# MetaHG/mitsuba2

Hardware: AMD Instinct MI355X
Metric: Msample/s, cbox 1024x1024@256spp per GPU, path integrator (max_depth=-1, rr_depth=5) (higher is better)
Workload: dtype f32

## Files before the change

### mitsuba2_amd/csrc/device_scene.h

```cpp
#pragma once
#include "device_math.h"
#include "device_bsdf.h"
#include "device_envmap.h"
#include "flat_worklist.h"

namespace mtsamd {

constexpr uint32_t kLeafFlag = 0x80000000u;
constexpr uint32_t kLeafCountShift = 27;
constexpr uint32_t kLeafStartMask = (1u << kLeafCountShift) - 1u;
constexpr uint32_t kNoPrim = 0xffffffffu;

#ifndef MTS_BVH4
#define MTS_BVH4 1
#endif
#if MTS_BVH4
typedef uint2 StackEntry;
typedef uint64_t StackRaw;
#else
typedef uint32_t StackEntry;
typedef uint32_t StackRaw;
#endif


struct DevShape { int32_t bsdf; int32_t emitter; uint32_t flags; uint32_t first_prim; };
constexpr uint32_t kShapeHasNormals = 1u, kShapeHasUV = 2u;
struct DevTexture {
    const float *data; int32_t w, h; uint32_t grad_offset, kind;
    float uvm[6];
    float c0[3], c1[3];
    float mean;
};
struct DevEmitter {
    float r, g, b; uint32_t shape;
    uint32_t first_prim, n_prims; float area_sum, area_norm;
    uint32_t valid_lo, valid_hi; uint32_t pad0, pad1;
    float c0, c1, c2, d65_scale;
// ... 22 lines not shown
    const float *tri_uv;
    const uint32_t *prim_shape;
    const DevShape *shapes;
    const DevBsdf *bsdfs;
    const DevEmitter *emitters; uint32_t n_emitters;
    uint32_t n_shapes, n_bsdfs;
    const DevTexture *textures; uint32_t n_textures;
    const float *area_pmf, *area_cdf;
    const float4 *flat_recs;
    const float4 *flat_pairs;
    uint32_t flat, n_pairs, n_clusters;
    int32_t env_emitter;
    const DevEnvmap *envmap;
    uint32_t general;
};
constexpr uint32_t kFlatMaxPrims = 64;

struct LdsView {
    const float4 *nodes;
    const float4 *tris;
    uint32_t *stack;
    uint32_t stride;
    StackEntry *spill;
    uint32_t spill_stride, stack_lds_depth;
    const float4 *flat;
    const float4 *pairs;
    const float4 *clusters;
    const DevShape *shapes;
    const DevBsdf *bsdfs;
    const DevEmitter *emitters;
    const float *pmf, *cdf;
    uint32_t *wl;
};

#ifndef MTS_FLAT_WORKLIST
#define MTS_FLAT_WORKLIST 1
#endif
#ifndef MTS_FLAT_WL_ROUNDS
#define MTS_FLAT_WL_ROUNDS 5
#endif
constexpr uint32_t kWlItems = 64u * MTS_FLAT_WL_ROUNDS;
constexpr uint32_t kWlWords = 128u + kWlItems / 2u;

inline uint32_t flat_shape_count(const SceneView &sv) { return sv.n_shapes; }

template <bool FLAT>
MTS_DEV LdsView lds_stage(const SceneView &sv, float4 *smem) {
    LdsView l = {};
    l.stride = blockDim.x;
    if (FLAT) {
        float4 *f = smem;
        for (uint32_t i = threadIdx.x; i < 4u * sv.n_prims; i += blockDim.x) f[i] = sv.flat_recs[i];
        l.flat = f;
        float4 *pr = f + 4u * sv.n_prims;
        for (uint32_t i = threadIdx.x; i < 5u * sv.n_pairs; i += blockDim.x) pr[i] = sv.flat_pairs[i];
        if (threadIdx.x < 5u) pr[5u * sv.n_pairs + threadIdx.x] = make_float4(0.0f, 0.0f, 0.0f, 0.0f);
        l.pairs = pr;
        float4 *cl = pr + 5u * sv.n_pairs + 5u;
        for (uint32_t i = threadIdx.x; i < 2u * sv.n_clusters; i += blockDim.x) cl[i] = sv.flat_pairs[5u * sv.n_pairs + i];
        l.clusters = cl;
        uint32_t *w = reinterpret_cast<uint32_t *>(cl + 2u * sv.n_clusters);
        const uint32_t n_sh = (sizeof(DevShape) / 4u) * sv.n_shapes, n_bs = (sizeof(DevBsdf) / 4u) * sv.n_bsdfs,
                       n_em = (sizeof(DevEmitter) / 4u) * sv.n_emitters;
        const uint32_t *g_sh = reinterpret_cast<const uint32_t *>(sv.shapes), *g_bs = reinterpret_cast<const uint32_t *>(sv.bsdfs),
                       *g_em = reinterpret_cast<const uint32_t *>(sv.emitters);
        for (uint32_t i = threadIdx.x; i < n_sh; i += blockDim.x) w[i] = g_sh[i];
        l.shapes = reinterpret_cast<const DevShape *>(w); w += n_sh;
        for (uint32_t i = threadIdx.x; i < n_bs; i += blockDim.x) w[i] = g_bs[i];
        l.bsdfs = reinterpret_cast<const DevBsdf *>(w); w += n_bs;
        for (uint32_t i = threadIdx.x; i < n_em; i += blockDim.x) w[i] = g_em[i];
        l.emitters = reinterpret_cast<const DevEmitter *>(w); w += n_em;
        float *fw = reinterpret_cast<float *>(w);
        for (uint32_t i = threadIdx.x; i < sv.n_prims; i += blockDim.x) { fw[i] = sv.area_pmf[i]; fw[sv.n_prims + i] = sv.area_cdf[i]; }
        l.pmf = fw; l.cdf = fw + sv.n_prims;
        const uint32_t wl_off = (uint32_t) (reinterpret_cast<uint32_t *>(fw + 2u * sv.n_prims) - reinterpret_cast<uint32_t *>(smem));
        l.wl = MTS_FLAT_WORKLIST ? reinterpret_cast<uint32_t *>(smem) + ((wl_off + 1u) & ~1u) : nullptr;
    } else {
        float4 *n = smem;
        float4 *t = n + 4u * sv.lds_nodes;
        for (uint32_t i = threadIdx.x; i < 4u * sv.lds_nodes; i += blockDim.x) n[i] = sv.nodes[i];
        for (uint32_t i = threadIdx.x; i < 3u * sv.lds_slots; i += blockDim.x) t[i] = sv.tris[i];
        l.nodes = n; l.tris = t;
        l.stack = reinterpret_cast<uint32_t *>(t + 3u * sv.lds_slots);
    }
    __syncthreads();
    return l;
}
inline size_t lds_bytes(const SceneView &sv, uint32_t block) {
    if (sv.flat)
        return (size_t) 64 * sv.n_prims + (size_t) 80 * (sv.n_pairs + 1) + (size_t) 32 * sv.n_clusters + sizeof(DevShape) * sv.n_shapes + sizeof(DevBsdf) * sv.n_bsdfs +
               sizeof(DevEmitter) * sv.n_emitters + (size_t) 8 * sv.n_prims +
               (MTS_FLAT_WORKLIST ? 4u + (size_t) 4 * kWlWords * (block / 64u) : 0u);
    return (size_t) 64 * sv.lds_nodes + (size_t) 48 * sv.lds_slots + sizeof(StackEntry) * sv.stack_depth * block;
}

#ifndef MTS_FLAT_UNROLL
#define MTS_FLAT_UNROLL 1
#endif
#ifndef MTS_FLAT_PREFETCH
#define MTS_FLAT_PREFETCH 1
#endif

struct Hit { float t; uint32_t prim; float u, v; };

MTS_DEV bool tri_test(f3 p0, f3 e1, f3 e2, f3 o, f3 d, float mint, float maxt, float &u, float &v, float &t) {
    f3 pvec = cross(d, e2);
    float inv_det = rcp(dot(e1, pvec));
    f3 tvec = o - p0;
    u = dot(tvec, pvec) * inv_det;
    bool ok = (u >= 0.0f) && (u <= 1.0f);
    f3 qvec = cross(tvec, e1);
    v = dot(d, qvec) * inv_det;
    ok = ok && (v >= 0.0f) && (u + v <= 1.0f);
    t = dot(e2, qvec) * inv_det;
    return ok && (t >= mint) && (t <= maxt);
}

MTS_DEV float clamp_mag(float r) { return fabsf(r) <= 3.0e38f ? r : copysignf(3.0e38f, r); }
MTS_DEV float clamp_mag33(float r) { return fabsf(r) <= 1.0e33f ? r : copysignf(1.0e33f, r); }
MTS_DEV float clamp_inv(float d) {
    float r = 1.0f / d;
    return fabsf(r) <= 3.0e38f ? r : copysignf(3.0e38f, d);
}

constexpr uint32_t kNoNode = 0x7fffffffu;
// ... 531 lines not shown
    if (MTS_FLAT_LATE_UV && best_prim != kNoPrim) flat_hit_uv(lds, o, d, best_prim, bu, bv);
    hit.t = best; hit.prim = best_prim; hit.u = bu; hit.v = bv;
    return best_prim != kNoPrim;
}

MTS_DEV bool traverse_flat_clustered_any(const SceneView &sv, const LdsView &lds, f3 o, f3 d, float mint, float maxt, uint32_t &tri_tests) {
    bool any = false;
    if (!(MTS_CULL_STATS & 2)) tri_tests += sv.n_prims;
    const v2f ox = splat(o.x), oy = splat(o.y), oz = splat(o.z), dx = splat(d.x), dy = splat(d.y), dz = splat(d.z);
    const f3 inv = mk3(clamp_inv(d.x), clamp_inv(d.y), clamp_inv(d.z));
    const float4 *rec = lds.pairs;
    for (uint32_t c = 0; c < sv.n_clusters; ++c) {
        const float4 lo = lds.clusters[2u * c], hi = lds.clusters[2u * c + 1u];
        const uint32_t n = __float_as_uint(lo.w);
        const float ax = (lo.x - o.x) * inv.x, bx = (hi.x - o.x) * inv.x;
        const float ay = (lo.y - o.y) * inv.y, by = (hi.y - o.y) * inv.y;
        const float az = (lo.z - o.z) * inv.z, bz = (hi.z - o.z) * inv.z;
        const float tn = fmaxf(fmaxf(fminf(ax, bx), fminf(ay, by)), fmaxf(fminf(az, bz), mint));
        const float tf = fminf(fminf(fmaxf(ax, bx), fmaxf(ay, by)), fminf(fmaxf(az, bz), maxt));
        if (__ballot(!any && tn <= tf) == 0ull) { rec += 5u * n; continue; }
        if (MTS_CULL_STATS & 2) tri_tests += 2u * n;
        for (uint32_t i = 0; i < n; ++i) {
            const float4 q0 = rec[0], q1 = rec[1], q2 = rec[2], q3 = rec[3], q4 = rec[4];
            rec += 5;
            const PairUvt r = pair_test(q0, q1, q2, q3, q4, ox, oy, oz, dx, dy, dz);
            const bool ok_a = tri_accept(r.u.x, r.v.x, r.uv.x, r.t.x, mint, maxt);
            const bool ok_b = tri_accept(r.u.y, r.v.y, r.uv.y, r.t.y, mint, maxt);
            any = any || ok_a || ok_b;
        }
    }
    return any;
}

static_assert(kFlatMaxPrims <= 64u, "a pair mask is 32 bits");
template <bool ANY>
MTS_DEV bool traverse_flat_worklist(const SceneView &sv, const LdsView &lds, f3 o, f3 d, float mint, float maxt, Hit &hit, uint32_t &tri_tests) {
    const uint64_t active = __ballot(1);
    const uint32_t n_act = (uint32_t) __popcll(active), lane = lane_id(), rank = mask_rank(active);
    const f3 inv = mk3(clamp_inv(d.x), clamp_inv(d.y), clamp_inv(d.z));
    uint32_t pairs = 0u, first = 0u;
    for (uint32_t c = 0; c < sv.n_clusters; ++c) {
        const float4 lo = lds.clusters[2u * c], hi = lds.clusters[2u * c + 1u];
        const uint32_t n = __float_as_uint(lo.w);
        const float ax = (lo.x - o.x) * inv.x, bx = (hi.x - o.x) * inv.x;
        const float ay = (lo.y - o.y) * inv.y, by = (hi.y - o.y) * inv.y;
        const float az = (lo.z - o.z) * inv.z, bz = (hi.z - o.z) * inv.z;
        const float tn = fmaxf(fmaxf(fminf(ax, bx), fminf(ay, by)), fmaxf(fminf(az, bz), mint));
        const float tf = fminf(fminf(fmaxf(ax, bx), fmaxf(ay, by)), fminf(fmaxf(az, bz), maxt));
        const uint32_t bits = (uint32_t) ((1ull << n) - 1ull) << first;
        pairs |= tn <= tf ? bits : 0u;
        first += n;
    }
    const uint32_t cnt = (uint32_t) __popc(pairs);
    uint32_t pos = 0u, total = 0u;
#pragma unroll
    for (uint32_t b = 0; b < 6u; ++b) {
        const uint64_t m = __ballot((cnt >> b) & 1u);
        pos += mask_rank(m) << b; total += (uint32_t) __popcll(m) << b;
    }
    if (total > kWlItems || total > MTS_FLAT_WL_ROUNDS * n_act) return traverse_flat<ANY>(sv, lds, o, d, mint, maxt, hit, tri_tests);
    constexpr bool kRealCount = (MTS_CULL_STATS & (ANY ? 2 : 1)) != 0;
    if (!kRealCount) tri_tests += sv.n_prims;
    uint32_t *ws = lds.wl + (threadIdx.x >> 6) * kWlWords;
    unsigned long long *key = reinterpret_cast<unsigned long long *>(ws);
    uint16_t *tbl = reinterpret_cast<uint16_t *>(ws + 128u);
    if (ANY) ws[lane] = 0u;
    else key[lane] = kWlNoKey;
    wl_push_items(tbl, pos, pairs, lane);
    __builtin_amdgcn_fence(__ATOMIC_RELEASE, "wavefront");
    __builtin_amdgcn_wave_barrier();
    __builtin_amdgcn_fence(__ATOMIC_ACQUIRE, "wavefront");
    for (uint32_t j0 = 0u; j0 < total; j0 += n_act) {
        const uint32_t j = j0 + rank;
        const uint32_t item = j < total ? (uint32_t) tbl[j] : wl_item(lane, sv.n_pairs);
        const uint32_t owner = wl_item_owner(item), pair = wl_item_pair(item);
        const int addr = (int) (owner << 2);
        const float rox = __int_as_float(__builtin_amdgcn_ds_bpermute(addr, __float_as_int(o.x)));
        const float roy = __int_as_float(__builtin_amdgcn_ds_bpermute(addr, __float_as_int(o.y)));
        const float roz = __int_as_float(__builtin_amdgcn_ds_bpermute(addr, __float_as_int(o.z)));
        const float rdx = __int_as_float(__builtin_amdgcn_ds_bpermute(addr, __float_as_int(d.x)));
        const float rdy = __int_as_float(__builtin_amdgcn_ds_bpermute(addr, __float_as_int(d.y)));
        const float rdz = __int_as_float(__builtin_amdgcn_ds_bpermute(addr, __float_as_int(d.z)));
        const float rmint = __int_as_float(__builtin_amdgcn_ds_bpermute(addr, __float_as_int(mint)));
        const float rmaxt = __int_as_float(__builtin_amdgcn_ds_bpermute(addr, __float_as_int(maxt)));
        const float4 *rec = lds.pairs + 5u * pair;
        const float4 q0 = rec[0], q1 = rec[1], q2 = rec[2], q3 = rec[3], q4 = rec[4];
        const PairUvt r = pair_test(q0, q1, q2, q3, q4, splat(rox), splat(roy), splat(roz), splat(rdx), splat(rdy), splat(rdz));
        const bool ok_a = tri_accept(r.u.x, r.v.x, r.uv.x, r.t.x, rmint, rmaxt);
        const bool ok_b = tri_accept(r.u.y, r.v.y, r.uv.y, r.t.y, rmint, rmaxt);
        if (kRealCount && j < total) tri_tests += 2u;
        if (ANY) {
            if (ok_a || ok_b) ws[owner] = 1u;
        } else if (ok_a || ok_b) {
            const uint64_t ka = ok_a ? wl_key(r.t.x, 2u * pair) : kWlNoKey, kb = ok_b ? wl_key(r.t.y, 2u * pair + 1u) : kWlNoKey;
            atomicMin(&key[owner], (unsigned long long) (ka < kb ? ka : kb));
        }
        if (ANY) {
            __builtin_amdgcn_fence(__ATOMIC_RELEASE, "wavefront");
            __builtin_amdgcn_wave_barrier();
            __builtin_amdgcn_fence(__ATOMIC_ACQUIRE, "wavefront");
            if (__ballot(ws[lane] == 0u && pos + cnt > j0 + n_act) == 0ull) break;
        }
    }
    __builtin_amdgcn_fence(__ATOMIC_RELEASE, "wavefront");
    __builtin_amdgcn_wave_barrier();
    __builtin_amdgcn_fence(__ATOMIC_ACQUIRE, "wavefront");
    if (ANY) return ws[lane] != 0u;
    const uint64_t k = key[lane];
    hit.t = maxt; hit.prim = kNoPrim; hit.u = 0.0f; hit.v = 0.0f;
    if (k == kWlNoKey) return false;
    hit.prim = wl_key_prim(k);
    hit.t = flat_hit_uv(lds, o, d, hit.prim, hit.u, hit.v);
    return true;
}

template <bool FLAT, bool ANY>
MTS_DEV bool traverse(const SceneView &sv, const LdsView &lds, f3 o, f3 d, float mint, float maxt, Hit &hit, uint32_t &tri_tests,
                      bool coherent = false) {
    if (FLAT && !ANY && MTS_FLAT_CULL && coherent && sv.n_clusters > 1u) return traverse_flat_clustered(sv, lds, o, d, mint, maxt, hit, tri_tests);
    if (FLAT && MTS_FLAT_WORKLIST && sv.n_clusters > 1u && lds.wl) return traverse_flat_worklist<ANY>(sv, lds, o, d, mint, maxt, hit, tri_tests);
    if (FLAT) return traverse_flat<ANY>(sv, lds, o, d, mint, maxt, hit, tri_tests);
    return traverse_bvh<ANY>(sv, lds, o, d, mint, maxt, hit, tri_tests);
}

template <bool ANY>
MTS_DEV bool traverse_naive(const SceneView &sv, f3 o, f3 d, float mint, float maxt, Hit &hit) {
    bool found = false; float best = maxt; uint32_t best_prim = kNoPrim;
    for (uint32_t s = 0; s < sv.n_slots; ++s) {
        const float4 *p = sv.tris + 3u * s;
        const float4 t0 = p[0], t1 = p[1], t2 = p[2];
        float u, v, t;
        if (tri_test(mk3(t0.x, t0.y, t0.z), mk3(t0.w, t1.x, t1.y), mk3(t1.z, t1.w, t2.x), o, d, mint, maxt, u, v, t)) {
            if (ANY) return true;
            uint32_t prim = __float_as_uint(t2.y);
// ... 324 lines not shown
```

### mitsuba2_amd/csrc/flat_worklist.h

```cpp
#pragma once
#include <cstdint>

namespace mtsamd {

constexpr uint32_t kWlPairShift = 6u;
__host__ __device__ inline uint32_t wl_item(uint32_t owner, uint32_t pair) { return pair << kWlPairShift | owner; }
__host__ __device__ inline uint32_t wl_item_owner(uint32_t item) { return item & 63u; }
__host__ __device__ inline uint32_t wl_item_pair(uint32_t item) { return item >> kWlPairShift; }

__host__ __device__ inline void wl_push_items(uint16_t *tbl, uint32_t pos, uint32_t pairs, uint32_t lane) {
    for (; pairs != 0u; pairs &= pairs - 1u, ++pos) tbl[pos] = (uint16_t) wl_item(lane, (uint32_t) __builtin_ctz(pairs));
}

constexpr uint64_t kWlNoKey = ~0ull;
__host__ __device__ inline uint32_t wl_t_order(float t) {
    const uint32_t b = t == 0.0f ? 0u : __builtin_bit_cast(uint32_t, t);
    return b ^ ((uint32_t) ((int32_t) b >> 31) | 0x80000000u);
}
__host__ __device__ inline uint64_t wl_key(float t, uint32_t prim) { return (uint64_t) wl_t_order(t) << 32 | (uint32_t) ~prim; }
__host__ __device__ inline uint32_t wl_key_prim(uint64_t key) { return ~(uint32_t) key; }

}
```

### mitsuba2_amd/csrc/kernels.h

```cpp
#pragma once
#include <hip/hip_runtime.h>
#include "device_scene.h"
#include "device_spectral.h"

namespace mtsamd {

struct PoolView {
    float4 *ray_o, *ray_d, *thr, *res;
    uint4 *rng;
    uint2 *misc;
    float *xi;
    float2 *aux;
    float4 *hit, *sh_o, *sh_d, *nee;
    uint32_t *sh_slot;
};

struct RowMap { int32_t row0, local_rows, tile_rows, part, count; };
MTS_DEV int32_t row_to_global(const RowMap &m, int32_t lr) {
    if (m.count <= 1) return m.row0 + lr;
    int32_t t = lr / m.tile_rows;
    return (t * m.count + m.part) * m.tile_rows + (lr - t * m.tile_rows);
}
MTS_DEV int32_t row_to_local(const RowMap &m, int32_t gr) {
    if (m.count <= 1) { int32_t lr = gr - m.row0; return (lr >= 0 && lr < m.local_rows) ? lr : -1; }
// ... 5 lines not shown
struct FilterView {
    float table[32];
    float radius, scale_factor, alpha, bias;
    int32_t kind, analytic, border, taps;
};

struct RenderParams {
    SceneView sv;
    CameraView cam;
    PoolView in, out;
    const uint32_t *count_in;
    uint32_t *count_out;
    uint32_t *count_shadow;
    uint64_t *cursor;
    const uint64_t *cursor_end;
    uint64_t *wave_stats;
    float4 *out_rgba;
    float2 *out_pos;
    uint32_t chunk;
    uint32_t n_chains;
    uint32_t first_pix, first_rem;
    uint64_t first_ordinal;
    uint64_t base_seed;
    RowMap rows;
    int32_t store_xyz;
    uint32_t plane_pix0, plane_pixels;
    uint32_t n_waves, seg_cap, target;
    int32_t spp, crop_x, crop_y, crop_w, crop_h;
    int32_t max_depth, rr_depth;
    int32_t spectral;
    int32_t integrator, emitter_samples, bsdf_samples, hide_emitters;
    int32_t split;
    uint32_t lds_queue_offset;
    uint32_t wave_first, wave_last;
    uint32_t gather_w;
    uint32_t trace_lds_depth;
    uint32_t trace_top_nodes;
    uint32_t *trace_spill;
};

constexpr uint32_t kMaxChains = 8u, kChainAlign = 64u;
constexpr uint32_t kTraceChains = 2u;
__host__ __device__ inline uint32_t chain_first(uint32_t k, uint32_t n, uint32_t chains) {
    if (k >= chains) return n;
    const uint32_t lo = ((uint32_t) ((uint64_t) n * k / chains) + kChainAlign - 1u) & ~(kChainAlign - 1u);
    return lo < n ? lo : n;
}
__host__ __device__ inline uint32_t chunk_owner(uint32_t wave, uint32_t n, uint32_t chains) {
    if (chains <= 1u) return wave;
    uint32_t s_min = n, k = 0u, lo_k = 0u, extra_before = 0u;
    for (uint32_t c = 0; c < chains; ++c) {
        const uint32_t lo = chain_first(c, n, chains), hi = chain_first(c + 1u, n, chains);
        s_min = hi - lo < s_min ? hi - lo : s_min;
        if (wave >= lo && wave < hi) { k = c; lo_k = lo; }
    }
    const uint32_t i = wave - lo_k;
    if (i < s_min) return i * chains + k;
    for (uint32_t c = 0; c < k; ++c) extra_before += chain_first(c + 1u, n, chains) - chain_first(c, n, chains) - s_min;
    return s_min * chains + extra_before + (i - s_min);
}

struct FilmParams {
    const float4 *out_rgba;
    const float2 *out_pos;
    float *film;
    FilterView filter;
// ... 69 lines not shown
```

### mitsuba2_amd/csrc/kernels.hip

```cpp
#include "kernels.h"

namespace mtsamd {

constexpr int kBlock = 256;

struct PathState {
    f3 o, d; float mint, maxt;
    f3 thr; float bs_pdf;
    f3 res; float eta;
    Pcg32 rng;
    uint32_t ordinal, depth, flags;
};

template <bool NT = false>
MTS_DEV void load_state(const PoolView &p, size_t i, PathState &s) {
    float4 a = ld_stream<NT>(p.ray_o + i), b = ld_stream<NT>(p.ray_d + i), c = ld_stream<NT>(p.thr + i), e = ld_stream<NT>(p.res + i);
    uint4 r = ld_stream<NT>(p.rng + i); uint2 m = ld_stream<NT>(p.misc + i);
    s.o = mk3(a.x, a.y, a.z); s.mint = a.w;
    s.d = mk3(b.x, b.y, b.z); s.maxt = b.w;
    s.thr = mk3(c.x, c.y, c.z); s.bs_pdf = c.w;
    s.res = mk3(e.x, e.y, e.z); s.eta = e.w;
    s.rng.state = (uint64_t) r.x | ((uint64_t) r.y << 32);
    s.rng.inc = (uint64_t) r.z | ((uint64_t) r.w << 32);
    s.ordinal = m.x; s.depth = m.y & 0xffffu; s.flags = m.y >> 16;
}
template <bool NT = false>
MTS_DEV void store_state(const PoolView &p, size_t i, const PathState &s) {
    st_stream<NT>(p.ray_o + i, make_float4(s.o.x, s.o.y, s.o.z, s.mint));
    st_stream<NT>(p.ray_d + i, make_float4(s.d.x, s.d.y, s.d.z, s.maxt));
    st_stream<NT>(p.thr + i, make_float4(s.thr.x, s.thr.y, s.thr.z, s.bs_pdf));
    p.res[i] = make_float4(s.res.x, s.res.y, s.res.z, s.eta);
    st_stream<NT>(p.rng + i, make_uint4((uint32_t) s.rng.state, (uint32_t) (s.rng.state >> 32), (uint32_t) s.rng.inc,
                                        (uint32_t) (s.rng.inc >> 32)));
// ... 822 lines not shown
        else hipLaunchKernelGGL((k_direct<false, false>), dim3(blocks), dim3(kBlock), lds, s, p, n);
    }
    return hipGetLastError();
}

constexpr uint32_t kFlagZombie = 2u;

template <bool GENERAL, bool FLAT>
MTS_DEV bool step_deferred(const RenderParams &P, const LdsView &lds, PathState &s, Counters &c, Deferred &df) {
    return bounce_step<FLAT, false, FLAT ? 2 : 1, GENERAL>(P, lds, s, c, nullptr, &df);
}
template <bool GENERAL, bool FLAT>
MTS_DEV bool step_deferred(const RenderParams &P, const LdsView &lds, PathStateS &s, Counters &c, Deferred &df) {
    return bounce_step_spectral<FLAT, FLAT ? 2 : 1, GENERAL>(P, lds, s, c, &df);
}
MTS_DEV void add_nee(PathState &s, const float (&nee)[4]) { s.res = mk3(s.res.x + nee[0], s.res.y + nee[1], s.res.z + nee[2]); }
MTS_DEV void add_nee(PathStateS &s, const float (&nee)[4]) {
#pragma unroll
    for (int k = 0; k < kWav; ++k) s.res.v[k] += nee[k];
}
MTS_DEV void finish_path(const RenderParams &P, const PathState &s) { store_result(P, s); }
MTS_DEV void finish_path(const RenderParams &P, const PathStateS &s) { store_result_spectral(P, s); }
MTS_DEV void start_path(const RenderParams &P, uint64_t ordinal, uint32_t lp, uint32_t j, PathState &s) { generate_path(P, ordinal, lp, j, s); }
MTS_DEV void start_path(const RenderParams &P, uint64_t ordinal, uint32_t lp, uint32_t j, PathStateS &s) { generate_path_spectral(P, ordinal, lp, j, s); }

#ifndef MTS_SHADE_WAVES_MIN
#define MTS_SHADE_WAVES_MIN 4
#endif
#ifndef MTS_SHADE_WAVES_MIN_RGB_DIFFUSE
#define MTS_SHADE_WAVES_MIN_RGB_DIFFUSE 5
#endif
template <typename State, bool GENERAL> struct ShadeWaves { static constexpr int kMin = MTS_SHADE_WAVES_MIN; };
template <> struct ShadeWaves<PathState, false> { static constexpr int kMin = MTS_SHADE_WAVES_MIN_RGB_DIFFUSE; };
constexpr uint32_t kShadowRing = 128u;
template <typename State> struct ShadowRing { float4 *o, *d, *nee; uint32_t *slot; };

template <typename State, bool GENERAL>
MTS_DEV void drain_shadow_ring(const RenderParams &P, const LdsView &lds, const ShadowRing<State> &q, uint32_t head, uint32_t count,
                               size_t base, Counters &c) {
    __builtin_amdgcn_fence(__ATOMIC_SEQ_CST, "workgroup");
    const uint32_t lane = lane_id();
    if (lane < count) {
        const uint32_t k = (head + lane) & (kShadowRing - 1u);
        const float4 o = q.o[k], d = q.d[k];
        Hit h;
        if (!traverse<true, true>(P.sv, lds, mk3(o.x, o.y, o.z), mk3(d.x, d.y, d.z), o.w, d.w, h, c.tri_tests)) {
            const size_t slot = base + q.slot[k];
            float4 r = P.out.res[slot];
            const float4 e = q.nee[k];
            r.x += e.x; r.y += e.y; r.z += e.z; r.w += e.w;
            P.out.res[slot] = r;
        }
    }
}

#ifndef MTS_NT_STREAMS
#define MTS_NT_STREAMS 3
#endif
#ifndef MTS_PRIMARY_SHADOW
#define MTS_PRIMARY_SHADOW 1
#endif
#ifndef MTS_SURV_ORDER
#define MTS_SURV_ORDER 1
#endif
template <typename State, bool GENERAL, bool FLAT, bool INLINE = false>
__global__ __launch_bounds__(kBlock) __attribute__((amdgpu_waves_per_eu(FLAT ? MTS_BOUNCE_WAVES : ShadeWaves<State, GENERAL>::kMin, FLAT ? MTS_BOUNCE_WAVES : 8)))
void k_shade(const RenderParams P) {
    static_assert(FLAT || !INLINE, "the in-kernel shadow queue is for LDS-resident scenes");
    constexpr bool kNT = !FLAT && (MTS_NT_STREAMS & 2) != 0;
    extern __shared__ float4 smem[];
    LdsView lds = {};
    const uint32_t gw = (FLAT && P.gather_w > 4u) ? P.gather_w : 4u;
    const uint32_t hw = threadIdx.x >> 6;
    const uint32_t wave = gw > 4u ? P.wave_first + blockIdx.x * gw + hw : P.wave_first + ((blockIdx.x * kBlock + threadIdx.x) >> 6);
    const uint32_t wave_last = P.wave_last ? P.wave_last : P.n_waves;
    __shared__ uint32_t s_cnt[kBlock / 64u], s_surv[kBlock / 64u];
    __shared__ uint32_t s_pre[FLAT ? 1025 : 1];
    if (FLAT && gw > 4u) {
        const uint32_t g0 = wave - hw;
        for (uint32_t k = threadIdx.x; k < gw; k += kBlock) s_pre[k + 1u] = (g0 + k < wave_last) ? P.count_in[g0 + k] : 0u;
        if (threadIdx.x == 0u) s_pre[0] = 0u;
        __syncthreads();
        if (hw == 0u) {
            const uint32_t per = (gw + 63u) / 64u, ln = lane_id();
            uint32_t local = 0u;
            for (uint32_t i = 0; i < per; ++i) { const uint32_t idx = ln * per + i; if (idx < gw) local += s_pre[idx + 1u]; }
            uint32_t incl = local;
            for (uint32_t off = 1u; off < 64u; off <<= 1) { const uint32_t v = __shfl_up(incl, off); if (ln >= off) incl += v; }
            uint32_t run = incl - local;
            for (uint32_t i = 0; i < per; ++i) { const uint32_t idx = ln * per + i; if (idx < gw) { run += s_pre[idx + 1u]; s_pre[idx + 1u] = run; } }
        }
        __syncthreads();
        if (s_pre[gw] == 0u) {
            for (uint32_t k = threadIdx.x; k < gw; k += kBlock) if (g0 + k < wave_last) P.count_out[g0 + k] = 0u;
            return;
        }
        lds = lds_stage<true>(P.sv, smem);
    } else if (FLAT) {
        const uint32_t n_own = wave < wave_last ? P.count_in[wave] : 0u;
        if (lane_id() == 0u) { s_cnt[threadIdx.x >> 6] = n_own; s_surv[threadIdx.x >> 6] = (wave < wave_last && MTS_SURV_ORDER) ? min(P.count_in[P.n_waves + wave], n_own) : 0u; }
        const bool work = wave < wave_last && (n_own > 0u || P.cursor[wave] < P.cursor_end[wave]);
        if (!__syncthreads_or(work ? 1 : 0)) {
            if (wave < wave_last && lane_id() == 0u) {
                P.count_out[wave] = 0u;
                if (!INLINE) P.count_shadow[wave] = 0u;
            }
            return;
        }
        lds = lds_stage<true>(P.sv, smem);
    }
    ShadowRing<State> ring = {};
    if (INLINE) {
        float4 *qb = smem + P.lds_queue_offset + (size_t) (threadIdx.x >> 6) * (kShadowRing * 13u / 4u);
        ring.o = qb; ring.d = qb + kShadowRing; ring.nee = qb + 2u * kShadowRing;
        ring.slot = reinterpret_cast<uint32_t *>(qb + 3u * kShadowRing);
    }
    if (wave >= wave_last) return;
    const uint32_t lane = lane_id();
    const size_t base = (size_t) wave * P.seg_cap;
    uint32_t n_out = 0;
    Counters c = { 0u, 0u, 0u, 0u };
    uint32_t n_sh = 0;
    uint32_t q_head = 0, q_count = 0;
    const uint32_t wg_wave0 = wave - (threadIdx.x >> 6);
    const uint32_t n_valid = FLAT ? min((uint32_t) (kBlock / 64u), wave_last - wg_wave0) : 1u;
    uint32_t reg[2u * (kBlock / 64u)], surv4[kBlock / 64u], n_in = 0;
    if (FLAT && gw > 4u) {
        n_in = s_pre[gw];
    } else if (FLAT) {
#pragma unroll
        for (uint32_t g = 0; g < kBlock / 64u; ++g) {
            const uint32_t cg = g < n_valid ? s_cnt[g] : 0u;
            surv4[g] = g < n_valid ? s_surv[g] : 0u;
            reg[g] = surv4[g]; reg[kBlock / 64u + g] = cg - surv4[g];
            n_in += cg;
        }
    } else {
        n_in = __builtin_amdgcn_readfirstlane(P.count_in[wave]);
    }

    for (uint32_t i0 = FLAT ? 64u * (threadIdx.x >> 6) : 0u; i0 < n_in; i0 += 64u * n_valid) {
        State s;
        Deferred df;
        df.pending = false;
        bool alive = false, zombie_now = false;
        uint32_t depth0 = 0u;
        if (i0 + lane < n_in) {
            size_t i = base + i0 + lane;
// ... 18 lines not shown
            if (s.flags & kFlagZombie) {
                finish_path(P, s);
            } else {
                depth0 = s.depth;
                if (!FLAT) {
                    const float4 h = ld_stream<kNT>(P.in.hit + i);
                    df.hit.t = h.x; df.hit.prim = __float_as_uint(h.y); df.hit.u = h.z; df.hit.v = h.w;
                    df.found = df.hit.prim != kNoPrim;
                }
                alive = step_deferred<GENERAL, FLAT>(P, lds, s, c, df);
                if (!alive) {
                    if (df.pending) { s.flags |= kFlagZombie; alive = true; zombie_now = true; }
                    else finish_path(P, s);
                }
            }
        }
        if (INLINE && MTS_FLAT_CULL && MTS_PRIMARY_SHADOW && P.sv.n_clusters > 1u && __ballot(depth0 != 1u && (i0 + lane < n_in)) == 0ull) {
            if (df.pending) {
                if (!traverse_flat_clustered_any(P.sv, lds, df.so, df.sd, df.smint, df.smaxt, c.tri_tests)) add_nee(s, df.nee);
                df.pending = false;
                if (zombie_now) { s.flags &= ~kFlagZombie; finish_path(P, s); alive = false; }
            }
        }
        const uint64_t m = __ballot(alive), ms = __ballot(alive && df.pending);
        if (alive) {
            const uint32_t slot = n_out + mask_rank(m);
            const size_t oidx = (FLAT && gw > 4u) ? ((size_t) wave + 4u * (slot / P.seg_cap)) * P.seg_cap + slot % P.seg_cap : base + slot;
            store_state<kNT>(P.out, oidx, s);
            if (df.pending) {
                if (INLINE) {
                    const uint32_t k = (q_head + q_count + mask_rank(ms)) & (kShadowRing - 1u);
                    ring.o[k] = make_float4(df.so.x, df.so.y, df.so.z, df.smint);
                    ring.d[k] = make_float4(df.sd.x, df.sd.y, df.sd.z, df.smaxt);
                    ring.nee[k] = make_float4(df.nee[0], df.nee[1], df.nee[2], df.nee[3]);
                    ring.slot[k] = (uint32_t) (oidx - base);
                } else {
                    const size_t q = base + n_sh + mask_rank(ms);
                    st_stream<kNT>(P.out.sh_o + q, make_float4(df.so.x, df.so.y, df.so.z, df.smint));
                    st_stream<kNT>(P.out.sh_d + q, make_float4(df.sd.x, df.sd.y, df.sd.z, df.smaxt));
                    st_stream<kNT>(P.out.nee + q, make_float4(df.nee[0], df.nee[1], df.nee[2], df.nee[3]));
                    st_stream<kNT>(P.out.sh_slot + q, slot);
                }
            }
        }
        n_out += (uint32_t) __popcll(m);
        n_sh += (uint32_t) __popcll(ms);
        if (INLINE) {
            q_count += (uint32_t) __popcll(ms);
            if (q_count >= 64u) {
                drain_shadow_ring<State, GENERAL>(P, lds, ring, q_head, 64u, base, c);
                q_head = (q_head + 64u) & (kShadowRing - 1u); q_count -= 64u;
            }
        }
    }
    if (INLINE && q_count > 0u) drain_shadow_ring<State, GENERAL>(P, lds, ring, q_head, q_count, base, c);

    const uint32_t n_surv = n_out;
    uint64_t cursor = P.cursor[wave];
    const uint64_t end = P.cursor_end[wave];
    while (n_out < P.target && cursor < end) {
        uint64_t left = end - cursor;
        uint32_t n_new = min(64u, P.target - n_out);
        if ((uint64_t) n_new > left) n_new = (uint32_t) left;
        if (lane < n_new) {
            State s;
            uint64_t ordinal; uint32_t lp, sj;
            cursor_sample(P, wave, cursor + lane, ordinal, lp, sj);
            start_path(P, ordinal, lp, sj, s);
// ... 310 lines not shown
                            k = item;
                        }
                    }
                }
            }
            if (__ballot(w.cur != kNoNode) == 0ull) {
                if (exhausted) break;
                continue;
            }
            MTS_PROF_MASK(ANY, exhausted ? 22 : 20, __ballot(w.cur != kNoNode));
            if (__ballot(w.cur != kNoNode && w.far) != 0ull) {
                if (w.cur != kNoNode) walk_round<ANY, true, kTraceTopNodes != 0u>(w, P.sv, st, tri_tests);
            } else {
                if (w.cur != kNoNode) walk_round<ANY, false, kTraceTopNodes != 0u>(w, P.sv, st, tri_tests);
            }
        }
    }
    for (int off = 32; off > 0; off >>= 1) tri_tests += __shfl_xor(tri_tests, off);
    if (lane_id() == 0 && tri_tests)
        atomicAdd(reinterpret_cast<unsigned long long *>(P.wave_stats + 4u * (size_t) w0 + 3u),
                  (unsigned long long) tri_tests);
}

#if MTS_TRACE_PROF
extern "C" __attribute__((visibility("default"))) int mtsamd_debug_trace_prof(unsigned long long *out, int reset) {
    static unsigned long long host[64 * 64];
    if (hipMemcpyFromSymbol(host, HIP_SYMBOL(g_trace_prof), sizeof(host)) != hipSuccess) return -1;
    for (int i = 0; i < 64; ++i) { out[i] = 0; for (int c = 0; c < 64; ++c) out[i] += host[64 * c + i]; }
    if (reset) { for (auto &h : host) h = 0; if (hipMemcpyToSymbol(HIP_SYMBOL(g_trace_prof), host, sizeof(host)) != hipSuccess) return -1; }
    return 0;
}
#endif

uint32_t trace_top_nodes(const SceneView &sv) { return std::min(sv.n_wnodes, kTraceTopNodes); }
uint32_t trace_group() { return kTraceGroup; }
size_t trace_lds_bytes(const SceneView &sv) {
    return (size_t) 64 * trace_top_nodes(sv) + sizeof(StackEntry) * (std::min(sv.stack_depth, kTraceLdsDepth) + 1u) * kTraceBlock;
}
uint32_t trace_lds_depth(const SceneView &sv) { return std::min(sv.stack_depth, kTraceLdsDepth); }
size_t trace_spill_words(const SceneView &sv, uint32_t n_waves) {
    const uint32_t spill = sv.stack_depth > kTraceLdsDepth ? sv.stack_depth - kTraceLdsDepth : 0u;
    const uint32_t spill_f = sv.stack_depth > kFinishLdsDepth ? sv.stack_depth - kFinishLdsDepth : 0u;
    const size_t trace = (size_t) 2 * ((n_waves + kTraceGroup - 1) / kTraceGroup) * spill * kTraceBlock;
    const size_t finish = (size_t) n_waves * spill_f * 64u;
    return (sizeof(StackEntry) / 4) * std::max(trace, finish);
}
static hipError_t allow_lds(const void *fn, size_t bytes) {
    return bytes > 48u * 1024u ? hipFuncSetAttribute(fn, hipFuncAttributeMaxDynamicSharedMemorySize, (int) bytes) : hipSuccess;
}

hipError_t launch_split_stage(const RenderParams &p, int stage, hipStream_t s) {
    const uint32_t n_launch = (p.wave_last ? p.wave_last : p.n_waves) - p.wave_first;
    const uint32_t shade_blocks = (n_launch * 64u + kBlock - 1) / kBlock, trace_blocks = (n_launch + kTraceGroup - 1) / kTraceGroup;
    if (stage == 0) {
        if (hipError_t e = allow_lds(reinterpret_cast<const void *>(&k_trace<false, false>), trace_lds_bytes(p.sv))) return e;
        hipLaunchKernelGGL((k_trace<false, false>), dim3(trace_blocks), dim3(kTraceBlock), trace_lds_bytes(p.sv), s, p);
    } else if (stage == 1) {
        if (p.spectral && p.sv.general) hipLaunchKernelGGL((k_shade<PathStateS, true, false>), dim3(shade_blocks), dim3(kBlock), 0, s, p);
        else if (p.spectral) hipLaunchKernelGGL((k_shade<PathStateS, false, false>), dim3(shade_blocks), dim3(kBlock), 0, s, p);
        else if (p.sv.general) hipLaunchKernelGGL((k_shade<PathState, true, false>), dim3(shade_blocks), dim3(kBlock), 0, s, p);
        else hipLaunchKernelGGL((k_shade<PathState, false, false>), dim3(shade_blocks), dim3(kBlock), 0, s, p);
    } else {
        if (hipError_t e = allow_lds(reinterpret_cast<const void *>(&k_trace<true, false>), trace_lds_bytes(p.sv))) return e;
        hipLaunchKernelGGL((k_trace<true, false>), dim3(trace_blocks), dim3(kTraceBlock), trace_lds_bytes(p.sv), s, p);
    }
    return hipGetLastError();
}

hipError_t launch_bounce(const RenderParams &p_, hipStream_t s) {
    RenderParams p = p_;
    if (p.split == 3) {
        const uint32_t n_launch = (p.wave_last ? p.wave_last : p.n_waves) - p.wave_first;
        const uint32_t shade_blocks = p.gather_w > 4u ? (n_launch + p.gather_w - 1u) / p.gather_w : (n_launch * 64u + kBlock - 1) / kBlock;
        const size_t scene_bytes = (bounce_lds_bytes(p.sv) + 15u) & ~(size_t) 15u;
        p.lds_queue_offset = (uint32_t) (scene_bytes / 16u);
        const size_t lds = scene_bytes + (size_t) (kBlock / 64u) * kShadowRing * 52u;
        if (p.spectral && p.sv.general) hipLaunchKernelGGL((k_shade<PathStateS, true, true, true>), dim3(shade_blocks), dim3(kBlock), lds, s, p);
        else if (p.spectral) hipLaunchKernelGGL((k_shade<PathStateS, false, true, true>), dim3(shade_blocks), dim3(kBlock), lds, s, p);
        else if (p.sv.general) hipLaunchKernelGGL((k_shade<PathState, true, true, true>), dim3(shade_blocks), dim3(kBlock), lds, s, p);
        else hipLaunchKernelGGL((k_shade<PathState, false, true, true>), dim3(shade_blocks), dim3(kBlock), lds, s, p);
        return hipGetLastError();
    }
    if (p.split == 2) {
        const uint32_t shade_blocks = (p.n_waves * 64u + kBlock - 1) / kBlock;
        const size_t lds = bounce_lds_bytes(p.sv);
        if (p.spectral && p.sv.general) hipLaunchKernelGGL((k_shade<PathStateS, true, true>), dim3(shade_blocks), dim3(kBlock), lds, s, p);
        else if (p.spectral) hipLaunchKernelGGL((k_shade<PathStateS, false, true>), dim3(shade_blocks), dim3(kBlock), lds, s, p);
        else if (p.sv.general) hipLaunchKernelGGL((k_shade<PathState, true, true>), dim3(shade_blocks), dim3(kBlock), lds, s, p);
        else hipLaunchKernelGGL((k_shade<PathState, false, true>), dim3(shade_blocks), dim3(kBlock), lds, s, p);
        hipLaunchKernelGGL((k_trace<true, true>), dim3((p.n_waves + kFlatGroup - 1) / kFlatGroup), dim3(kBlock), lds, s, p);
        return hipGetLastError();
    }
    if (p.split) {
        hipError_t e = launch_split_stage(p, 0, s);
        if (e == hipSuccess) e = launch_split_stage(p, 1, s);
        if (e == hipSuccess) e = launch_split_stage(p, 2, s);
        return e;
    }
    uint32_t blocks = (p.n_waves * 64u + kBlock - 1) / kBlock;
    if (p.spectral) {
        if (p.sv.general == 2u) {
            if (p.sv.flat) hipLaunchKernelGGL((k_bounce_spectral<true, true, true>), dim3(blocks), dim3(kBlock), bounce_lds_bytes(p.sv), s, p);
            else hipLaunchKernelGGL((k_bounce_spectral<false, true, true>), dim3(blocks), dim3(kBlock), bounce_lds_bytes(p.sv), s, p);
        } else if (p.sv.general) {
            if (p.sv.flat) hipLaunchKernelGGL((k_bounce_spectral<true, true>), dim3(blocks), dim3(kBlock), bounce_lds_bytes(p.sv), s, p);
            else hipLaunchKernelGGL((k_bounce_spectral<false, true>), dim3(blocks), dim3(kBlock), bounce_lds_bytes(p.sv), s, p);
        } else {
            if (p.sv.flat) hipLaunchKernelGGL((k_bounce_spectral<true, false>), dim3(blocks), dim3(kBlock), bounce_lds_bytes(p.sv), s, p);
            else hipLaunchKernelGGL((k_bounce_spectral<false, false>), dim3(blocks), dim3(kBlock), bounce_lds_bytes(p.sv), s, p);
// ... 891 lines not shown
```

Measured before the change: 3722.

## Window the flat work-list, pack shadow-ring slot into NEE, move prefix scratch to dynamic LDS

The flat-scene work-list now runs in windows of up to a configurable item count (default 1024) with a round cap. This replaces the old 5-round limit that sent waves to the per-lane brute-force traversal. For RGB the shadow ring stores the output slot in the unused w lane of the NEE record, which shrinks each ring entry from 52 to 48 bytes. The static prefix-sum scratch array moves into the dynamically sized LDS layout, computed by a shared helper. Together these aim for fewer fallback traversals and a smaller LDS footprint. The trade-off is that the larger work-list window raises per-wave LDS, which could lower occupancy.

```diff
diff --git a/mitsuba2_amd/csrc/device_scene.h b/mitsuba2_amd/csrc/device_scene.h
--- a/mitsuba2_amd/csrc/device_scene.h
+++ b/mitsuba2_amd/csrc/device_scene.h
@@ -3,6 +3,7 @@
 #include "device_bsdf.h"
 #include "device_envmap.h"
 #include "flat_worklist.h"
+#include "flat_lds.h"
 
 namespace mtsamd {
 
@@ -91,15 +92,6 @@
     const float *pmf, *cdf;
     uint32_t *wl;
 };
-
-#ifndef MTS_FLAT_WORKLIST
-#define MTS_FLAT_WORKLIST 1
-#endif
-#ifndef MTS_FLAT_WL_ROUNDS
-#define MTS_FLAT_WL_ROUNDS 5
-#endif
-constexpr uint32_t kWlItems = 64u * MTS_FLAT_WL_ROUNDS;
-constexpr uint32_t kWlWords = 128u + kWlItems / 2u;
 
 inline uint32_t flat_shape_count(const SceneView &sv) { return sv.n_shapes; }
 
@@ -145,11 +137,16 @@
     __syncthreads();
     return l;
 }
+__host__ __device__ inline uint32_t flat_table_bytes(uint32_t n_prims, uint32_t n_pairs, uint32_t n_clusters, uint32_t n_shapes, uint32_t n_bsdfs,
+                                                     uint32_t n_emitters) {
+    return 64u * n_prims + 80u * (n_pairs + 1u) + 32u * n_clusters + (uint32_t) sizeof(DevShape) * n_shapes + (uint32_t) sizeof(DevBsdf) * n_bsdfs +
+           (uint32_t) sizeof(DevEmitter) * n_emitters + 8u * n_prims;
+}
+inline uint32_t flat_table_bytes(const SceneView &sv) {
+    return flat_table_bytes(sv.n_prims, sv.n_pairs, sv.n_clusters, sv.n_shapes, sv.n_bsdfs, sv.n_emitters);
+}
 inline size_t lds_bytes(const SceneView &sv, uint32_t block) {
-    if (sv.flat)
-        return (size_t) 64 * sv.n_prims + (size_t) 80 * (sv.n_pairs + 1) + (size_t) 32 * sv.n_clusters + sizeof(DevShape) * sv.n_shapes + sizeof(DevBsdf) * sv.n_bsdfs +
-               sizeof(DevEmitter) * sv.n_emitters + (size_t) 8 * sv.n_prims +
-               (MTS_FLAT_WORKLIST ? 4u + (size_t) 4 * kWlWords * (block / 64u) : 0u);
+    if (sv.flat) return flat_lds_layout(flat_table_bytes(sv), block / 64u, 0u, 0u).ring;
     return (size_t) 64 * sv.lds_nodes + (size_t) 48 * sv.lds_slots + sizeof(StackEntry) * sv.stack_depth * block;
 }
 
@@ -747,6 +744,9 @@
     return any;
 }
 
+#if MTS_CULL_STATS
+static __device__ unsigned long long g_wl_fallback[2];
+#endif
 static_assert(kFlatMaxPrims <= 64u, "a pair mask is 32 bits");
 template <bool ANY>
 MTS_DEV bool traverse_flat_worklist(const SceneView &sv, const LdsView &lds, f3 o, f3 d, float mint, float maxt, Hit &hit, uint32_t &tri_tests) {
@@ -773,7 +773,12 @@
         const uint64_t m = __ballot((cnt >> b) & 1u);
         pos += mask_rank(m) << b; total += (uint32_t) __popcll(m) << b;
     }
-    if (total > kWlItems || total > MTS_FLAT_WL_ROUNDS * n_act) return traverse_flat<ANY>(sv, lds, o, d, mint, maxt, hit, tri_tests);
+    if (wl_rounds(total, n_act) > MTS_FLAT_WL_MAX_ROUNDS) {
+#if MTS_CULL_STATS
+        if (rank == 0u) atomicAdd(&g_wl_fallback[ANY ? 1 : 0], (unsigned long long) n_act);
+#endif
+        return traverse_flat<ANY>(sv, lds, o, d, mint, maxt, hit, tri_tests);
+    }
     constexpr bool kRealCount = (MTS_CULL_STATS & (ANY ? 2 : 1)) != 0;
     if (!kRealCount) tri_tests += sv.n_prims;
     uint32_t *ws = lds.wl + (threadIdx.x >> 6) * kWlWords;
@@ -781,40 +786,51 @@
     uint16_t *tbl = reinterpret_cast<uint16_t *>(ws + 128u);
     if (ANY) ws[lane] = 0u;
     else key[lane] = kWlNoKey;
-    wl_push_items(tbl, pos, pairs, lane);
-    __builtin_amdgcn_fence(__ATOMIC_RELEASE, "wavefront");
-    __builtin_amdgcn_wave_barrier();
-    __builtin_amdgcn_fence(__ATOMIC_ACQUIRE, "wavefront");
-    for (uint32_t j0 = 0u; j0 < total; j0 += n_act) {
-        const uint32_t j = j0 + rank;
-        const uint32_t item = j < total ? (uint32_t) tbl[j] : wl_item(lane, sv.n_pairs);
-        const uint32_t owner = wl_item_owner(item), pair = wl_item_pair(item);
-        const int addr = (int) (owner << 2);
-        const float rox = __int_as_float(__builtin_amdgcn_ds_bpermute(addr, __float_as_int(o.x)));
-        const float roy = __int_as_float(__builtin_amdgcn_ds_bpermute(addr, __float_as_int(o.y)));
-        const float roz = __int_as_float(__builtin_amdgcn_ds_bpermute(addr, __float_as_int(o.z)));
-        const float rdx = __int_as_float(__builtin_amdgcn_ds_bpermute(addr, __float_as_int(d.x)));
-        const float rdy = __int_as_float(__builtin_amdgcn_ds_bpermute(addr, __float_as_int(d.y)));
-        const float rdz = __int_as_float(__builtin_amdgcn_ds_bpermute(addr, __float_as_int(d.z)));
-        const float rmint = __int_as_float(__builtin_amdgcn_ds_bpermute(addr, __float_as_int(mint)));
-        const float rmaxt = __int_as_float(__builtin_amdgcn_ds_bpermute(addr, __float_as_int(maxt)));
-        const float4 *rec = lds.pairs + 5u * pair;
-        const float4 q0 = rec[0], q1 = rec[1], q2 = rec[2], q3 = rec[3], q4 = rec[4];
-        const PairUvt r = pair_test(q0, q1, q2, q3, q4, splat(rox), splat(roy), splat(roz), splat(rdx), splat(rdy), splat(rdz));
-        const bool ok_a = tri_accept(r.u.x, r.v.x, r.uv.x, r.t.x, rmint, rmaxt);
-        const bool ok_b = tri_accept(r.u.y, r.v.y, r.uv.y, r.t.y, rmint, rmaxt);
-        if (kRealCount && j < total) tri_tests += 2u;
-        if (ANY) {
-            if (ok_a || ok_b) ws[owner] = 1u;
-        } else if (ok_a || ok_b) {
-            const uint64_t ka = ok_a ? wl_key(r.t.x, 2u * pair) : kWlNoKey, kb = ok_b ? wl_key(r.t.y, 2u * pair + 1u) : kWlNoKey;
-            atomicMin(&key[owner], (unsigned long long) (ka < kb ? ka : kb));
-        }
-        if (ANY) {
+    const uint32_t wn = wl_window(kWlItems, n_act);
+    bool done = false;
+    for (uint32_t w0 = 0u; w0 < total && !done; w0 += wn) {
+        if (w0 > 0u) {
             __builtin_amdgcn_fence(__ATOMIC_RELEASE, "wavefront");
             __builtin_amdgcn_wave_barrier();
             __builtin_amdgcn_fence(__ATOMIC_ACQUIRE, "wavefront");
-            if (__ballot(ws[lane] == 0u && pos + cnt > j0 + n_act) == 0ull) break;
+        }
+        if (total <= wn) wl_push_items(tbl, pos, pairs, lane);
+        else wl_push_window(tbl, pos, pairs, lane, w0, wn);
+        __builtin_amdgcn_fence(__ATOMIC_RELEASE, "wavefront");
+        __builtin_amdgcn_wave_barrier();
+        __builtin_amdgcn_fence(__ATOMIC_ACQUIRE, "wavefront");
+        const uint32_t w_end = min(total, w0 + wn);
+        for (uint32_t j0 = w0; j0 < w_end; j0 += n_act) {
+            const uint32_t j = j0 + rank;
+            const uint32_t item = j < total ? (uint32_t) tbl[j - w0] : wl_item(lane, sv.n_pairs);
+            const uint32_t owner = wl_item_owner(item), pair = wl_item_pair(item);
+            const int addr = (int) (owner << 2);
+            const float rox = __int_as_float(__builtin_amdgcn_ds_bpermute(addr, __float_as_int(o.x)));
+            const float roy = __int_as_float(__builtin_amdgcn_ds_bpermute(addr, __float_as_int(o.y)));
+            const float roz = __int_as_float(__builtin_amdgcn_ds_bpermute(addr, __float_as_int(o.z)));
+            const float rdx = __int_as_float(__builtin_amdgcn_ds_bpermute(addr, __float_as_int(d.x)));
+            const float rdy = __int_as_float(__builtin_amdgcn_ds_bpermute(addr, __float_as_int(d.y)));
+            const float rdz = __int_as_float(__builtin_amdgcn_ds_bpermute(addr, __float_as_int(d.z)));
+            const float rmint = __int_as_float(__builtin_amdgcn_ds_bpermute(addr, __float_as_int(mint)));
+            const float rmaxt = __int_as_float(__builtin_amdgcn_ds_bpermute(addr, __float_as_int(maxt)));
+            const float4 *rec = lds.pairs + 5u * pair;
+            const float4 q0 = rec[0], q1 = rec[1], q2 = rec[2], q3 = rec[3], q4 = rec[4];
+            const PairUvt r = pair_test(q0, q1, q2, q3, q4, splat(rox), splat(roy), splat(roz), splat(rdx), splat(rdy), splat(rdz));
+            const bool ok_a = tri_accept(r.u.x, r.v.x, r.uv.x, r.t.x, rmint, rmaxt);
+            const bool ok_b = tri_accept(r.u.y, r.v.y, r.uv.y, r.t.y, rmint, rmaxt);
+            if (kRealCount && j < total) tri_tests += 2u;
+            if (ANY) {
+                if (ok_a || ok_b) ws[owner] = 1u;
+            } else if (ok_a || ok_b) {
+                const uint64_t ka = ok_a ? wl_key(r.t.x, 2u * pair) : kWlNoKey, kb = ok_b ? wl_key(r.t.y, 2u * pair + 1u) : kWlNoKey;
+                atomicMin(&key[owner], (unsigned long long) (ka < kb ? ka : kb));
+            }
+            if (ANY) {
+                __builtin_amdgcn_fence(__ATOMIC_RELEASE, "wavefront");
+                __builtin_amdgcn_wave_barrier();
+                __builtin_amdgcn_fence(__ATOMIC_ACQUIRE, "wavefront");
+                if (__ballot(ws[lane] == 0u && pos + cnt > j0 + n_act) == 0ull) { done = true; break; }
+            }
         }
     }
     __builtin_amdgcn_fence(__ATOMIC_RELEASE, "wavefront");
diff --git a/mitsuba2_amd/csrc/flat_lds.h b/mitsuba2_amd/csrc/flat_lds.h
--- /dev/null
+++ b/mitsuba2_amd/csrc/flat_lds.h
@@ -0,0 +1,38 @@
+#pragma once
+#include <cstdint>
+
+namespace mtsamd {
+
+#ifndef MTS_FLAT_WORKLIST
+#define MTS_FLAT_WORKLIST 1
+#endif
+#ifndef MTS_FLAT_WL_WINDOW
+#define MTS_FLAT_WL_WINDOW 1024
+#endif
+#ifndef MTS_FLAT_WL_MAX_ROUNDS
+#define MTS_FLAT_WL_MAX_ROUNDS 32
+#endif
+constexpr uint32_t kWlItems = MTS_FLAT_WL_WINDOW;
+static_assert(kWlItems >= 64u && kWlItems % 64u == 0u, "the work-list window holds whole rounds of a full wave");
+constexpr uint32_t kWlWords = 128u + kWlItems / 2u;
+
+constexpr uint32_t kShadowRing = 128u;
+constexpr uint32_t kShadowRingEntryRgb = 48u, kShadowRingEntrySpectral = 52u;
+
+struct FlatLds {
+    uint32_t wl;
+    uint32_t ring;
+    uint32_t pre;
+    uint32_t bytes;
+};
+__host__ __device__ inline FlatLds flat_lds_layout(uint32_t table_bytes, uint32_t waves, uint32_t ring_entry, uint32_t pre_words) {
+    FlatLds l;
+    l.wl = (table_bytes + 7u) & ~7u;
+    const uint32_t wl_end = l.wl + (MTS_FLAT_WORKLIST ? 4u * kWlWords * waves : 0u);
+    l.ring = (wl_end + 15u) & ~15u;
+    l.pre = l.ring + waves * kShadowRing * ring_entry;
+    l.bytes = l.pre + 4u * pre_words;
+    return l;
+}
+
+}
diff --git a/mitsuba2_amd/csrc/flat_worklist.h b/mitsuba2_amd/csrc/flat_worklist.h
--- a/mitsuba2_amd/csrc/flat_worklist.h
+++ b/mitsuba2_amd/csrc/flat_worklist.h
@@ -12,6 +12,13 @@
     for (; pairs != 0u; pairs &= pairs - 1u, ++pos) tbl[pos] = (uint16_t) wl_item(lane, (uint32_t) __builtin_ctz(pairs));
 }
 
+__host__ __device__ inline uint32_t wl_window(uint32_t cap, uint32_t n_act) { return n_act * (cap / n_act); }
+__host__ __device__ inline uint32_t wl_rounds(uint32_t items, uint32_t n_act) { return (items + n_act - 1u) / n_act; }
+__host__ __device__ inline void wl_push_window(uint16_t *tbl, uint32_t pos, uint32_t pairs, uint32_t lane, uint32_t w0, uint32_t wn) {
+    for (; pairs != 0u; pairs &= pairs - 1u, ++pos)
+        if (pos - w0 < wn) tbl[pos - w0] = (uint16_t) wl_item(lane, (uint32_t) __builtin_ctz(pairs));
+}
+
 constexpr uint64_t kWlNoKey = ~0ull;
 __host__ __device__ inline uint32_t wl_t_order(float t) {
     const uint32_t b = t == 0.0f ? 0u : __builtin_bit_cast(uint32_t, t);
diff --git a/mitsuba2_amd/csrc/kernels.h b/mitsuba2_amd/csrc/kernels.h
--- a/mitsuba2_amd/csrc/kernels.h
+++ b/mitsuba2_amd/csrc/kernels.h
@@ -61,6 +61,7 @@
     int32_t integrator, emitter_samples, bsdf_samples, hide_emitters;
     int32_t split;
     uint32_t lds_queue_offset;
+    uint32_t lds_pre_offset;
     uint32_t wave_first, wave_last;
     uint32_t gather_w;
     uint32_t trace_lds_depth;
diff --git a/mitsuba2_amd/csrc/kernels.hip b/mitsuba2_amd/csrc/kernels.hip
--- a/mitsuba2_amd/csrc/kernels.hip
+++ b/mitsuba2_amd/csrc/kernels.hip
@@ -1,4 +1,5 @@
 #include "kernels.h"
+#include <type_traits>
 
 namespace mtsamd {
 
@@ -887,8 +888,11 @@
 #endif
 template <typename State, bool GENERAL> struct ShadeWaves { static constexpr int kMin = MTS_SHADE_WAVES_MIN; };
 template <> struct ShadeWaves<PathState, false> { static constexpr int kMin = MTS_SHADE_WAVES_MIN_RGB_DIFFUSE; };
-constexpr uint32_t kShadowRing = 128u;
-template <typename State> struct ShadowRing { float4 *o, *d, *nee; uint32_t *slot; };
+template <typename State> struct ShadowRing {
+    static constexpr bool kSlotInNee = std::is_same<State, PathState>::value;
+    static constexpr uint32_t kEntry = kSlotInNee ? kShadowRingEntryRgb : kShadowRingEntrySpectral;
+    float4 *o, *d, *nee; uint32_t *slot;
+};
 
 template <typename State, bool GENERAL>
 MTS_DEV void drain_shadow_ring(const RenderParams &P, const LdsView &lds, const ShadowRing<State> &q, uint32_t head, uint32_t count,
@@ -900,10 +904,10 @@
         const float4 o = q.o[k], d = q.d[k];
         Hit h;
         if (!traverse<true, true>(P.sv, lds, mk3(o.x, o.y, o.z), mk3(d.x, d.y, d.z), o.w, d.w, h, c.tri_tests)) {
-            const size_t slot = base + q.slot[k];
+            const float4 e = q.nee[k];
+            const size_t slot = base + (ShadowRing<State>::kSlotInNee ? __float_as_uint(e.w) : q.slot[k]);
             float4 r = P.out.res[slot];
-            const float4 e = q.nee[k];
-            r.x += e.x; r.y += e.y; r.z += e.z; r.w += e.w;
+            r.x += e.x; r.y += e.y; r.z += e.z; r.w += ShadowRing<State>::kSlotInNee ? 0.0f : e.w;
             P.out.res[slot] = r;
         }
     }
@@ -930,7 +934,7 @@
     const uint32_t wave = gw > 4u ? P.wave_first + blockIdx.x * gw + hw : P.wave_first + ((blockIdx.x * kBlock + threadIdx.x) >> 6);
     const uint32_t wave_last = P.wave_last ? P.wave_last : P.n_waves;
     __shared__ uint32_t s_cnt[kBlock / 64u], s_surv[kBlock / 64u];
-    __shared__ uint32_t s_pre[FLAT ? 1025 : 1];
+    uint32_t *s_pre = reinterpret_cast<uint32_t *>(smem + P.lds_pre_offset);
     if (FLAT && gw > 4u) {
         const uint32_t g0 = wave - hw;
         for (uint32_t k = threadIdx.x; k < gw; k += kBlock) s_pre[k + 1u] = (g0 + k < wave_last) ? P.count_in[g0 + k] : 0u;
@@ -966,9 +970,9 @@
     }
     ShadowRing<State> ring = {};
     if (INLINE) {
-        float4 *qb = smem + P.lds_queue_offset + (size_t) (threadIdx.x >> 6) * (kShadowRing * 13u / 4u);
+        float4 *qb = smem + P.lds_queue_offset + (size_t) (threadIdx.x >> 6) * (kShadowRing * ShadowRing<State>::kEntry / 16u);
         ring.o = qb; ring.d = qb + kShadowRing; ring.nee = qb + 2u * kShadowRing;
-        ring.slot = reinterpret_cast<uint32_t *>(qb + 3u * kShadowRing);
+        ring.slot = ShadowRing<State>::kSlotInNee ? nullptr : reinterpret_cast<uint32_t *>(qb + 3u * kShadowRing);
     }
     if (wave >= wave_last) return;
     const uint32_t lane = lane_id();
@@ -1053,8 +1057,13 @@
                     const uint32_t k = (q_head + q_count + mask_rank(ms)) & (kShadowRing - 1u);
                     ring.o[k] = make_float4(df.so.x, df.so.y, df.so.z, df.smint);
                     ring.d[k] = make_float4(df.sd.x, df.sd.y, df.sd.z, df.smaxt);
-                    ring.nee[k] = make_float4(df.nee[0], df.nee[1], df.nee[2], df.nee[3]);
-                    ring.slot[k] = (uint32_t) (oidx - base);
+                    const uint32_t rs = (uint32_t) (oidx - base);
+                    if (ShadowRing<State>::kSlotInNee) {
+                        ring.nee[k] = make_float4(df.nee[0], df.nee[1], df.nee[2], __uint_as_float(rs));
+                    } else {
+                        ring.nee[k] = make_float4(df.nee[0], df.nee[1], df.nee[2], df.nee[3]);
+                        ring.slot[k] = rs;
+                    }
                 } else {
                     const size_t q = base + n_sh + mask_rank(ms);
                     st_stream<kNT>(P.out.sh_o + q, make_float4(df.so.x, df.so.y, df.so.z, df.smint));
@@ -1431,6 +1440,15 @@
 }
 #endif
 
+#if MTS_CULL_STATS
+extern "C" __attribute__((visibility("default"))) int mtsamd_debug_wl_fallback(unsigned long long *out2, int reset) {
+    if (hipMemcpyFromSymbol(out2, HIP_SYMBOL(g_wl_fallback), 2 * sizeof(unsigned long long)) != hipSuccess) return -1;
+    const unsigned long long zero[2] = { 0ull, 0ull };
+    if (reset && hipMemcpyToSymbol(HIP_SYMBOL(g_wl_fallback), zero, sizeof(zero)) != hipSuccess) return -1;
+    return 0;
+}
+#endif
+
 uint32_t trace_top_nodes(const SceneView &sv) { return std::min(sv.n_wnodes, kTraceTopNodes); }
 uint32_t trace_group() { return kTraceGroup; }
 size_t trace_lds_bytes(const SceneView &sv) {
@@ -1471,9 +1489,14 @@
     if (p.split == 3) {
         const uint32_t n_launch = (p.wave_last ? p.wave_last : p.n_waves) - p.wave_first;
         const uint32_t shade_blocks = p.gather_w > 4u ? (n_launch + p.gather_w - 1u) / p.gather_w : (n_launch * 64u + kBlock - 1) / kBlock;
-        const size_t scene_bytes = (bounce_lds_bytes(p.sv) + 15u) & ~(size_t) 15u;
-        p.lds_queue_offset = (uint32_t) (scene_bytes / 16u);
-        const size_t lds = scene_bytes + (size_t) (kBlock / 64u) * kShadowRing * 52u;
+        const FlatLds l = flat_lds_layout(flat_table_bytes(p.sv), kBlock / 64u, p.spectral ? kShadowRingEntrySpectral : kShadowRingEntryRgb,
+                                          p.gather_w > 4u ? p.gather_w + 1u : 0u);
+        p.lds_queue_offset = l.ring / 16u;
+        p.lds_pre_offset = l.pre / 16u;
+        const size_t lds = l.bytes;
+        const void *fn = p.spectral ? (p.sv.general ? reinterpret_cast<const void *>(&k_shade<PathStateS, true, true, true>) : reinterpret_cast<const void *>(&k_shade<PathStateS, false, true, true>))
+                                    : (p.sv.general ? reinterpret_cast<const void *>(&k_shade<PathState, true, true, true>) : reinterpret_cast<const void *>(&k_shade<PathState, false, true, true>));
+        if (hipError_t e = allow_lds(fn, lds)) return e;
         if (p.spectral && p.sv.general) hipLaunchKernelGGL((k_shade<PathStateS, true, true, true>), dim3(shade_blocks), dim3(kBlock), lds, s, p);
         else if (p.spectral) hipLaunchKernelGGL((k_shade<PathStateS, false, true, true>), dim3(shade_blocks), dim3(kBlock), lds, s, p);
         else if (p.sv.general) hipLaunchKernelGGL((k_shade<PathState, true, true, true>), dim3(shade_blocks), dim3(kBlock), lds, s, p);
```

Result: no change. 3720 (median of 4 runs) (-0.1%).
